# pmeletis/IV2019-boosting-semantic-segmentation-with-weak-labels

Hardware: NVIDIA B200
Metric: train_images_per_s (higher is better)
Workload: dtype bf16

## Files before the change

include/wlseg.h:

```cpp
#ifndef WLSEG_H_
#define WLSEG_H_

#include <stddef.h>
#include <stdint.h>

#ifdef __cplusplus
extern "C" {
#endif

#define WLSEG_VERSION 100

typedef void* wlseg_stream_t;

enum { WLSEG_F32 = 0, WLSEG_BF16 = 1 };
enum { WLSEG_ALGO_AUTO = 0, WLSEG_ALGO_DIRECT = 1, WLSEG_ALGO_TCGEN05 = 2 };

int wlseg_version(void);
const char* wlseg_last_error(void);

typedef struct wlseg_conv_params {
  int32_t N, H, W, C;
  int32_t K, R, S;
  int32_t P, Q;
  int32_t stride, dilation;
// ... 59 lines not shown

int wlseg_bn_finalize_apply(const double* sum, const double* sqsum, int64_t count, int32_t C,
                            const float* gamma, const float* beta, float eps, float decay,
                            float* moving_mean, float* moving_var, float* scale, float* shift,
                            float* saved_mean, float* saved_invstd, const void* z, const void* residual,
                            void* y, uint8_t* relu_mask, int32_t relu, int32_t dtype, wlseg_stream_t stream);

int wlseg_bn_apply(const void* z, const float* scale, const float* shift, const void* residual,
                   void* y, int64_t count, int32_t C, int32_t relu, int32_t dtype,
                   wlseg_stream_t stream);

int wlseg_bn_apply_mask(const void* z, const float* scale, const float* shift, const void* residual,
                        void* y, uint8_t* relu_mask, int64_t count, int32_t C, int32_t dtype,
                        wlseg_stream_t stream);

int wlseg_bn_bwd_reduce(const void* dy, const void* y, const void* z, const float* mean,
                        const float* invstd, const float* scale, const float* shift, int64_t count,
                        int32_t C, int32_t pitch, int32_t relu, int32_t dtype, double* dgamma,
                        double* dbeta, wlseg_stream_t stream);
int wlseg_bn_bwd_apply(const void* dy, const void* y, const void* z, const float* mean,
                       const float* invstd, const float* gamma, const float* scale, const float* shift,
                       const double* dgamma, const double* dbeta, int64_t count, int64_t stat_count,
                       int32_t C, int32_t pitch, int32_t relu, int32_t dtype, void* dz, void* dres,
                       wlseg_stream_t stream);

int wlseg_maxpool_same_fwd(const void* x, void* y, uint8_t* argmax, int32_t N, int32_t H, int32_t W,
                           int32_t C, int32_t ksize, int32_t stride, int32_t dtype,
                           wlseg_stream_t stream);
int wlseg_maxpool_same_bwd(const void* x, const uint8_t* argmax, const void* dy, void* dx, int32_t N,
                           int32_t H, int32_t W, int32_t C, int32_t ksize, int32_t stride,
                           int32_t dtype, wlseg_stream_t stream);

int wlseg_gn_finalize(const double* sum, const double* sqsum, int32_t N, int32_t C, int32_t groups, int64_t hw,
                      const float* gamma, const float* beta, float eps, float* scale, float* shift, float* mean,
                      float* invstd, wlseg_stream_t stream);
int wlseg_gn_bwd_finalize(const double* dgamma_nc, const double* dbeta_nc, int32_t N, int32_t C, int32_t groups,
                          int64_t hw, const float* gamma, const float* mean, const float* invstd, float* cA,
                          float* c1, float* c0, double* dgamma, double* dbeta, wlseg_stream_t stream);
int wlseg_gn_bwd_apply(const void* dy, const void* y, const void* z, const float* cA, const float* c1,
                       const float* c0, const float* scale, const float* shift, int32_t N, int64_t hw, int32_t C,
                       int32_t relu, int32_t dtype, void* dz, void* dres, wlseg_stream_t stream);

int wlseg_avgpool_valid_fwd(const void* x, void* y, int32_t N, int32_t H, int32_t W, int32_t C, int32_t kh,
// ... 106 lines not shown
```

iv2019-boosting-semantic-segmentation-with-weak-labels_b200/csrc/bn.cu:

```cuda
#include <cstdlib>

#include "common.cuh"

namespace wlseg {

static int env_int(const char* name, int dflt) {
  const char* e = getenv(name);
  return e ? atoi(e) : dflt;
}

constexpr int kBnThreads = 256;
constexpr int kBnUnroll = 4;

template <typename T, bool kBackward>
__global__ void __launch_bounds__(kBnThreads)
bn_reduce_kernel(const T* __restrict__ a, const T* __restrict__ yact, const T* __restrict__ z,
                 const float* __restrict__ mean, const float* __restrict__ invstd, const float* __restrict__ scale,
                 const float* __restrict__ shift, int64_t count, int C, int pitch, int relu,
                 double* __restrict__ out0, double* __restrict__ out1, int cspan, int rev) {
  extern __shared__ float part[];
  pdl_launch_dependents();
  pdl_wait();
  if (cspan < C) {
    const int cb = blockIdx.y * cspan;
// ... 290 lines not shown
struct BnFin {
  const double* sum;
  const double* sqsum;
  const float* gamma;
  const float* beta;
  float* moving_mean;
  float* moving_var;
  float* scale_out;
  float* shift_out;
  float* saved_mean;
  float* saved_invstd;
  int64_t count;
  float eps, decay;
};

template <typename T, int kRowsU>
__global__ void __launch_bounds__(256)
bn_apply_rows_kernel(const T* __restrict__ z, const float* __restrict__ scale, const float* __restrict__ shift,
                     const T* __restrict__ res, T* __restrict__ y, int64_t count, int C, int relu, int rev,
                     uint8_t* __restrict__ relu_mask, const BnFin fin) {
  pdl_launch_dependents();
  pdl_wait();
  const int cv = C / 8;
  const int lanes = 256 / cv;
  const int tx = threadIdx.x % cv, ty = threadIdx.x / cv;
  if (ty >= lanes) return;
  const int c0 = tx * 8;
  float sc[8], sh[8];
  if (fin.sum != nullptr) {
    const double n = (double)fin.count;
    const bool publish = blockIdx.x == 0 && ty == 0;
#pragma unroll
    for (int j = 0; j < 8; ++j) {
      const int c = c0 + j;
      const double m = fin.sum[c] / n;
// ... 9 lines not shown
        fin.saved_mean[c] = mf;
        fin.saved_invstd[c] = inv;
        if (fin.moving_mean != nullptr) {
          const float unbiased = fin.count > 1 ? (float)(var * (n / (n - 1.0))) : vf;
          fin.moving_mean[c] -= (1.0f - fin.decay) * (fin.moving_mean[c] - mf);
          fin.moving_var[c] -= (1.0f - fin.decay) * (fin.moving_var[c] - unbiased);
        }
      }
    }
  } else {
    const float4 sa = *reinterpret_cast<const float4*>(scale + c0), sb = *reinterpret_cast<const float4*>(scale + c0 + 4);
    const float4 ha = *reinterpret_cast<const float4*>(shift + c0), hb = *reinterpret_cast<const float4*>(shift + c0 + 4);
    sc[0] = sa.x; sc[1] = sa.y; sc[2] = sa.z; sc[3] = sa.w; sc[4] = sb.x; sc[5] = sb.y; sc[6] = sb.z; sc[7] = sb.w;
    sh[0] = ha.x; sh[1] = ha.y; sh[2] = ha.z; sh[3] = ha.w; sh[4] = hb.x; sh[5] = hb.y; sh[6] = hb.z; sh[7] = hb.w;
  }
  const int64_t step = (int64_t)gridDim.x * lanes;
  for (int64_t row0 = (int64_t)blockIdx.x * lanes + ty; row0 < count; row0 += step * kRowsU) {
    Vec8<T> v[kRowsU], vr[kRowsU];
#pragma unroll
    for (int u = 0; u < kRowsU; ++u) {
      const int64_t row = row0 + u * step;
      if (row < count) {
        const int64_t r = rev ? count - 1 - row : row;
        v[u].load(z + r * C + c0);
        if (res != nullptr) vr[u].load(res + r * C + c0);
      }
    }
#pragma unroll
    for (int u = 0; u < kRowsU; ++u) {
      int64_t row = row0 + u * step;
      if (row >= count) break;
      if (rev) row = count - 1 - row;
      float f[8];
      v[u].unpack(f);
#pragma unroll
      for (int j = 0; j < 8; ++j) f[j] = f[j] * sc[j] + sh[j];
      if (res != nullptr) {
        float r[8];
        vr[u].unpack(r);
#pragma unroll
        for (int j = 0; j < 8; ++j) f[j] += r[j];
      }
      if (relu) {
#pragma unroll
        for (int j = 0; j < 8; ++j) f[j] = fmaxf(f[j], 0.f);
      }
      Vec8<T> o;
      o.pack(f);
      o.store(y + row * C + c0);
      if (relu_mask != nullptr) {
        uint32_t m = 0;
#pragma unroll
        for (int j = 0; j < 8; ++j) m |= (f[j] > 0.f ? 1u : 0u) << j;
        relu_mask[row * cv + tx] = (uint8_t)m;
// ... 71 lines not shown
      Vec8<T> o;
      o.pack(out);
      o.store(dz + e);
    }
  }
}

static bool bn_rows_enabled() { return getenv("WLSEG_BN_FLAT") == nullptr; }
static int bn_apply_u() { return env_int("WLSEG_BN_APPLY_U", 2); }
static int bn_apply_ctas() { return env_int("WLSEG_BN_APPLY_CTAS", 4); }
static int bn_bwd_u() { return env_int("WLSEG_BN_BWD_U", 2); }
static int bn_bwd_ctas() { return env_int("WLSEG_BN_BWD_CTAS", 2); }

template <typename T>
static void launch_apply_rows(const void* z, const float* scale, const float* shift, const void* res, void* y, int64_t count,
                              int C, int relu, cudaStream_t s, uint8_t* mask = nullptr, const BnFin* finp = nullptr) {
  BnFin fin = {};
  if (finp != nullptr) fin = *finp;
  const int lanes = 256 / (C / 8);
  const int U = res != nullptr ? bn_apply_u() : env_int("WLSEG_BN_APPLY_U_PLAIN", 1);
  const int g = bw_grid(ceil_div(count, (int64_t)lanes * U) * 256, 256,
                        res != nullptr ? bn_apply_ctas() : env_int("WLSEG_BN_APPLY_CTAS_PLAIN", 8));
  const int rev = env_int("WLSEG_BN_APPLY_REV", 1);
  cudaError_t e;
  if (U == 1) e = launch_pdl(bn_apply_rows_kernel<T, 1>, dim3(g), dim3(256), 0, s, (const T*)z, scale, shift, (const T*)res, (T*)y, count, C, relu, rev, mask, fin);
  else if (U == 4) e = launch_pdl(bn_apply_rows_kernel<T, 4>, dim3(g), dim3(256), 0, s, (const T*)z, scale, shift, (const T*)res, (T*)y, count, C, relu, rev, mask, fin);
  else e = launch_pdl(bn_apply_rows_kernel<T, 2>, dim3(g), dim3(256), 0, s, (const T*)z, scale, shift, (const T*)res, (T*)y, count, C, relu, rev, mask, fin);
  (void)e;
}

template <typename T>
static void launch_bwd_apply_rows(const void* dy, const void* y, const void* z, const float* mean, const float* invstd,
                                  const float* gamma, const float* scale, const float* shift, const double* dgamma,
                                  const double* dbeta, int64_t count, int64_t stat_count, int C, int pitch, int relu,
                                  void* dz, void* dres, cudaStream_t s) {
  const int lanes = 256 / (C / 8);
  const int U = bn_bwd_u();
  const int g = bw_grid(ceil_div(count, (int64_t)lanes * U) * 256, 256, bn_bwd_ctas());
#define WLSEG_BWD_ROWS(UU)                                                                                          \
  (void)launch_pdl(bn_bwd_apply_rows_kernel<T, UU>, dim3(g), dim3(256), 0, s, (const T*)dy, (const T*)y, (const T*)z,  \
                   mean, invstd, gamma, scale, shift, dgamma, dbeta, count, stat_count, C, pitch, relu, (T*)dz,        \
                   (T*)dres)
// ... 204 lines not shown
  else
    WLSEG_CHECK_ARG(false, "bn_apply: bad dtype %d", dtype);
  WLSEG_LAUNCH_CHECK();
  return 0;
}

extern "C" int wlseg_bn_apply_mask(const void* z, const float* scale, const float* shift, const void* residual, void* y,
                                   uint8_t* relu_mask, int64_t count, int32_t C, int32_t dtype, wlseg_stream_t stream) {
  if (int e = check_bn_shape(count, C, "bn_apply_mask")) return e;
  if (count == 0) return 0;
  WLSEG_CHECK_ARG(z && scale && shift && y && relu_mask, "bn_apply_mask: null pointer");
  WLSEG_CHECK_ARG(C % 32 == 0 && C <= 2048, "bn_apply_mask: C must be a multiple of 32 and <= 2048 (got %d)", C);
  if (dtype == WLSEG_BF16) launch_apply_rows<__nv_bfloat16>(z, scale, shift, residual, y, count, C, 1, (cudaStream_t)stream, relu_mask);
  else if (dtype == WLSEG_F32) launch_apply_rows<float>(z, scale, shift, residual, y, count, C, 1, (cudaStream_t)stream, relu_mask);
  else WLSEG_CHECK_ARG(false, "bn_apply_mask: bad dtype %d", dtype);
  WLSEG_LAUNCH_CHECK();
  return 0;
}

extern "C" int wlseg_bn_bwd_reduce(const void* dy, const void* y, const void* z, const float* mean,
                                   const float* invstd, const float* scale, const float* shift, int64_t count,
                                   int32_t C, int32_t pitch, int32_t relu, int32_t dtype, double* dgamma,
                                   double* dbeta, wlseg_stream_t stream) {
  if (int e = check_bn_shape(count, C, "bn_bwd_reduce")) return e;
  if (count == 0) return 0;
  WLSEG_CHECK_ARG(dy && z && mean && invstd && dgamma && dbeta && (!relu || y || (scale && shift)),
                  "bn_bwd_reduce: null pointer");
  WLSEG_CHECK_ARG(pitch >= C && (C % 8 != 0 ? pitch == C : pitch % 8 == 0), "bn_bwd_reduce: bad pitch %d", pitch);
  WLSEG_CHECK_ARG(C % 8 == 0 || !relu || y, "bn_bwd_reduce: the small-C path needs y for the ReLU mask");
  if (dtype == WLSEG_BF16)
// ... 64 lines not shown
```

iv2019-boosting-semantic-segmentation-with-weak-labels_b200/csrc/pool.cu:

```cuda
#include <cstdlib>

#include "common.cuh"

namespace wlseg {

struct PoolGeom {
  int N, H, W, C, P, Q, k, stride, pad_t, pad_l;
};

template <typename T>
__global__ void __launch_bounds__(256)
maxpool_fwd_kernel(const T* __restrict__ x, T* __restrict__ y, uint8_t* __restrict__ argmax, PoolGeom g) {
  const int cv = g.C / 8;
  const int64_t total = (int64_t)g.N * g.P * g.Q * cv;
  for (int64_t i = (int64_t)blockIdx.x * blockDim.x + threadIdx.x; i < total; i += (int64_t)gridDim.x * blockDim.x) {
    int c8 = (int)(i % cv);
    int64_t t = i / cv;
    int q = (int)(t % g.Q); t /= g.Q;
    int p = (int)(t % g.P);
    int n = (int)(t / g.P);
    float best[8];
    uint32_t arg[8];
#pragma unroll
    for (int j = 0; j < 8; ++j) { best[j] = -INFINITY; arg[j] = 255u; }
// ... 17 lines not shown
    Vec8<T> o;
    o.pack(best);
    const int64_t oi = (((int64_t)n * g.P + p) * g.Q + q) * g.C + c8 * 8;
    o.store(y + oi);
    if (argmax != nullptr) {
      uint2 packed;
      packed.x = arg[0] | (arg[1] << 8) | (arg[2] << 16) | (arg[3] << 24);
      packed.y = arg[4] | (arg[5] << 8) | (arg[6] << 16) | (arg[7] << 24);
      *reinterpret_cast<uint2*>(argmax + oi) = packed;
    }
  }
}

constexpr int kPoolRun = 4;

template <typename T>
__global__ void __launch_bounds__(256)
maxpool3x3s2_fwd_kernel(const T* __restrict__ x, T* __restrict__ y, uint8_t* __restrict__ argmax, PoolGeom g) {
  const int cv = g.C / 8;
  const int runs = (g.Q + kPoolRun - 1) / kPoolRun;
  const int64_t total = (int64_t)g.N * g.P * runs * cv;
  for (int64_t i = (int64_t)blockIdx.x * blockDim.x + threadIdx.x; i < total; i += (int64_t)gridDim.x * blockDim.x) {
    const int c8 = (int)(i % cv);
    int64_t t = i / cv;
    const int run = (int)(t % runs); t /= runs;
    const int p = (int)(t % g.P);
    const int n = (int)(t / g.P);
    const int q0 = run * kPoolRun;
    const int h0 = p * 2 - g.pad_t;
    const T* base = x + (int64_t)n * g.H * g.W * g.C + c8 * 8;
    Vec8<T> col[3][3];
    bool okc[3], okr[3];
#pragma unroll
    for (int r = 0; r < 3; ++r) okr[r] = (h0 + r >= 0) && (h0 + r < g.H);
    auto load_col = [&](int ww, int slot) {
      okc[slot] = ww >= 0 && ww < g.W;
#pragma unroll
      for (int r = 0; r < 3; ++r)
        if (okc[slot] && okr[r]) col[slot][r].load(base + ((int64_t)(h0 + r) * g.W + ww) * g.C);
    };
    const int w0 = q0 * 2 - g.pad_l;
    load_col(w0, 0);
#pragma unroll
    for (int u = 0; u < kPoolRun; ++u) {
      const int q = q0 + u;
      if (q >= g.Q) break;
      const int ww = q * 2 - g.pad_l;
      load_col(ww + 1, 1);
      load_col(ww + 2, 2);
      float best[8];
      uint32_t arg[8];
#pragma unroll
      for (int j = 0; j < 8; ++j) { best[j] = -INFINITY; arg[j] = 255u; }
#pragma unroll
// ... 209 lines not shown

using namespace wlseg;

extern "C" int wlseg_maxpool_same_fwd(const void* x, void* y, uint8_t* argmax, int32_t N, int32_t H, int32_t W,
                                      int32_t C, int32_t ksize, int32_t stride, int32_t dtype,
                                      wlseg_stream_t stream) {
  PoolGeom g;
  if (int e = make_geom(g, N, H, W, C, ksize, stride)) return e;
  if (N == 0) return 0;
  WLSEG_CHECK_ARG(x && y, "maxpool_fwd: null pointer");
  WLSEG_CHECK_ARG(argmax == nullptr || ksize * ksize < 255, "maxpool_fwd: window too large for the uint8 argmax map");
  if (ksize == 3 && stride == 2 && getenv("WLSEG_POOL_GENERIC") == nullptr) {
    const int64_t items3 = (int64_t)N * g.P * ((g.Q + kPoolRun - 1) / kPoolRun) * (C / 8);
    const int grid3 = bw_grid(items3, 256, 2);
    if (dtype == WLSEG_BF16)
      maxpool3x3s2_fwd_kernel<<<grid3, 256, 0, (cudaStream_t)stream>>>((const __nv_bfloat16*)x, (__nv_bfloat16*)y, argmax, g);
    else if (dtype == WLSEG_F32)
      maxpool3x3s2_fwd_kernel<<<grid3, 256, 0, (cudaStream_t)stream>>>((const float*)x, (float*)y, argmax, g);
    else
      WLSEG_CHECK_ARG(false, "maxpool_fwd: bad dtype %d", dtype);
    WLSEG_LAUNCH_CHECK();
    return 0;
  }
  int64_t items = (int64_t)N * g.P * g.Q * (C / 8);
  int grid = bw_grid(items, 256, 8);
  if (dtype == WLSEG_BF16)
    maxpool_fwd_kernel<<<grid, 256, 0, (cudaStream_t)stream>>>((const __nv_bfloat16*)x, (__nv_bfloat16*)y, argmax, g);
  else if (dtype == WLSEG_F32)
    maxpool_fwd_kernel<<<grid, 256, 0, (cudaStream_t)stream>>>((const float*)x, (float*)y, argmax, g);
  else
    WLSEG_CHECK_ARG(false, "maxpool_fwd: bad dtype %d", dtype);
  WLSEG_LAUNCH_CHECK();
  return 0;
}

extern "C" int wlseg_maxpool_same_bwd(const void* x, const uint8_t* argmax, const void* dy, void* dx, int32_t N,
                                      int32_t H, int32_t W, int32_t C, int32_t ksize, int32_t stride,
                                      int32_t dtype, wlseg_stream_t stream) {
  PoolGeom g;
  if (int e = make_geom(g, N, H, W, C, ksize, stride)) return e;
  if (N == 0) return 0;
  WLSEG_CHECK_ARG((x || argmax) && dy && dx, "maxpool_bwd: null pointer");
  int64_t items = (int64_t)N * H * W * (C / 8);
  int grid = bw_grid(items, 256, 8);
  const bool rows_ok = H <= 65535 && N <= 65535 && getenv("WLSEG_POOL_FLAT") == nullptr;
  const dim3 rgrid((unsigned)ceil_div((int64_t)W * (C / 8), 256), (unsigned)H, (unsigned)N);
// ... 43 lines not shown
```

iv2019-boosting-semantic-segmentation-with-weak-labels_b200/wlseg/network.py:

```python

import math
import os

import torch

from wlseg import arch, ops


def _trunc_normal_(t, std, gen):
  torch.nn.init.trunc_normal_(t, mean=0.0, std=std, a=-2 * std, b=2 * std, generator=gen)


class Params:

  def __init__(self, hier, device, output_stride=8, psp=False, fov=None, upsampling='bilinear', norm='batch'):
    self.hier = hier
    self.device = torch.device(device)
    self.psp = bool(psp)
    self.fov = tuple(fov) if fov and fov[0] > 0 and fov[1] > 0 else None
    if upsampling not in ('bilinear', 'no', 'hybrid'):
      raise ValueError('No such upsampling method.')
    self.upsampling = upsampling
    self.specs = arch.conv_specs(hier.head_widths, output_stride, psp=self.psp, fov=self.fov, upsampling=upsampling)
    self.plain = set(arch.UPSAMPLING_SCOPES) if upsampling == 'hybrid' else set()
# ... 558 lines not shown
               cross_replica=None):
    super().__init__(params, dtype, bn_decay, eps, conv_algo)
    self.ws = TrainWorkspace(params)
    self.cross_replica = cross_replica if (cross_replica and cross_replica[0] >= 1) else None
    self.grad_ready = None
    self.keep = False
    self._flipped = None
    self.fused_bn_finalize = os.environ.get('WLSEG_BN_FUSED_FINALIZE', '0') == '1'
    self.bn_bwd_l2_bytes = 1 << 40
    self._order = {s.scope: i for i, s in enumerate(params.specs)}
    self.wgrad_stream = None
    self._side_keep = []
    self.premask = os.environ.get('WLSEG_RELU_MASK', '1') != '0'
    self.bnb_fuse = os.environ.get('WLSEG_BNB_FUSE', '1') != '0'
    self.fin_in_conv = os.environ.get('WLSEG_BN_FIN_IN_CONV', '0') == '1'

  def _mark_done(self, scope, n_elems):
    if self.grad_ready is None:
      return
    lo = self.p.w_off[scope]
    i = self._order[scope]
    specs = self.p.specs
    while i < len(specs) and self.p.w_off[specs[i].scope] < lo + n_elems:
      self._done[i] = True
      i += 1
    t = self._tail
    while t > 0 and self._done[t - 1]:
      t -= 1
    if t != self._tail:
      self._tail = t
      self.grad_ready(self.p.w_off[specs[t].scope])

  def _layer_fwd(self, x, scope, *, w=None, nch=None, relu=None, residual=None, pad=None, stride=None,
                 dilation=None, out_hw=None, y_f32=False, kind='conv', want_mask=False):
    spec = self.p.by_scope[scope]
    if w is None:
      w = self._weights(scope)
    K = w.shape[0] if nch is None else nch
    if pad is None:
      pt, pl, P, Q = self._geom(spec, x.shape[1], x.shape[2])
      pad, out_hw, stride, dilation = (pt, pl), (P, Q), spec.stride, spec.dilation
    N = x.shape[0]
    count = N * out_hw[0] * out_hw[1]
    ws, off = self.ws, self.p.c_off[scope]
    s1, s2 = ws.view(ws.stat, 0, off, K), ws.view(ws.stat, 1, off, K)
    zdt = torch.float32 if y_f32 else self.dtype
    group = self.p.norm == 'group'
    scale, shift = ws.view(ws.bn, 0, off, K), ws.view(ws.bn, 1, off, K)
    mean, invstd = ws.view(ws.bn, 2, off, K), ws.view(ws.bn, 3, off, K)
    fin = None
    if (self.fin_in_conv and not group and self.cross_replica is None and not self.fused_bn_finalize and not y_f32 and
        self.dtype == torch.bfloat16 and self.conv_algo != ops.ALGO_DIRECT and K % 64 == 0 and x.shape[3] % 8 == 0 and
        x.stride(2) % 8 == 0 and not ops.pdl_enabled()):
      fin = (count, self.p.gamma(scope, K), self.p.beta(scope, K), self.eps, self.bn_decay, self.p.moving_mean(scope, K),
             self.p.moving_var(scope, K), scale, shift, mean, invstd, ws.fin_counter)
    z = self._conv(x, w, stride=stride, dilation=dilation, pad=pad, out_hw=out_hw, y_dtype=zdt,
                   bn_sum=None if group else s1, bn_sqsum=None if group else s2, fin=fin)
    a = torch.empty_like(z)
    do_relu = spec.relu if relu is None else relu
    gn = None
    mask = None
    if group:
      gn = self._gn_forward(z, scope, K, do_relu, residual, a)
    elif self.cross_replica is not None:
      R = self.cross_replica[0]
      both = self._all_reduce_pair(s1, s2)
      ops.bn_finalize(both[:K], both[K:], count * R, K, self.p.gamma(scope, K), self.p.beta(scope, K), self.eps,
                      self.bn_decay, self.p.moving_mean(scope, K), self.p.moving_var(scope, K), scale, shift, mean,
                      invstd, moving_var_factor=(count - 1.0) / count)
      ops.bn_apply(z, scale, shift, residual, a, count, K, do_relu)
    elif self.fused_bn_finalize and K % 8 == 0 and K <= 2048 and z.is_contiguous():
      if want_mask and do_relu and K % 32 == 0:
        mask = torch.empty((count, K // 8), dtype=torch.uint8, device=self.dev)
      ops.bn_finalize_apply(s1, s2, count, K, self.p.gamma(scope, K), self.p.beta(scope, K), self.eps, self.bn_decay,
                            self.p.moving_mean(scope, K), self.p.moving_var(scope, K), scale, shift, mean, invstd,
                            z, residual, a, do_relu, mask=mask)
    else:
      if fin is None:
        ops.bn_finalize(s1, s2, count, K, self.p.gamma(scope, K), self.p.beta(scope, K), self.eps, self.bn_decay,
                        self.p.moving_mean(scope, K), self.p.moving_var(scope, K), scale, shift, mean, invstd)
      if want_mask and do_relu and K % 32 == 0 and K <= 2048 and z.is_contiguous():
        mask = torch.empty((count, K // 8), dtype=torch.uint8, device=self.dev)
      ops.bn_apply(z, scale, shift, residual, a, count, K, do_relu, mask=mask)
    rec = _Rec()
    rec.scope, rec.spec, rec.x, rec.w, rec.z, rec.a = scope, spec, x, w, z, a
    rec.relu, rec.has_res, rec.geom, rec.nch, rec.kind = do_relu, residual is not None, (pad, out_hw, stride, dilation), K, kind
    rec.gn = gn
    rec.mask = mask
    rec.res = residual if self.keep else None
    self.tape[scope] = rec
    return a

  def _gn_forward(self, z, scope, K, relu, residual, a):
    N, P, Q, _ = z.shape
    hw = P * Q
    sums = torch.zeros((2, N, K), dtype=torch.float64, device=self.dev)
    for n in range(N):
      ops.bn_stats(z[n], hw, K, z.stride(2), sums[0, n], sums[1, n])
    coef = torch.empty((4, N, K), dtype=torch.float32, device=self.dev)
    ops.gn_finalize(sums[0], sums[1], N, K, self.p.groups(scope, K), hw, self.p.gamma(scope, K), self.p.beta(scope, K),
                    self.eps, coef[0], coef[1], coef[2], coef[3])
    for n in range(N):
      ops.bn_apply(z[n], coef[0, n], coef[1, n], None if residual is None else residual[n], a[n], hw, K, relu)
    return coef

  def _gn_backward(self, rec, da, scope, K, dgamma, dbeta):
# ... 174 lines not shown
        assert dx.is_contiguous()
        ops.add_inplace(dx, dx_add)
    if self.keep:
      rec.dx = dx
    return dx, dres

  def _root_fwd(self, images):
    scope = f'{arch.RES}/conv1'
    N, H, W, _ = images.shape
    if self.dtype == torch.bfloat16:
      Hs, Ws = (H + 1) // 2, (W + 1) // 2
      packed = torch.empty((N, Hs, Ws, 64), dtype=torch.bfloat16, device=self.dev)
      ops.conv1_pack(images, packed)
      self._root_images = images
      y = self._layer_fwd(packed, scope, w=self.p.conv1_packed_weights(torch.bfloat16), pad=(2, 0), stride=1,
                          dilation=1, out_hw=(Hs, Ws), relu=True, kind='root_packed')
    else:
      y = self._layer_fwd(images.to(self.dtype), scope)
    P, Q = (y.shape[1] + 1) // 2, (y.shape[2] + 1) // 2
    pooled = torch.empty((N, P, Q, 64), dtype=self.dtype, device=self.dev)
    amax = torch.empty((N, P, Q, 64), dtype=torch.uint8, device=self.dev)
    ops.maxpool_same_fwd(y, pooled, 3, 2, argmax=amax)
    self.tape['pool1'] = (y, amax)
    return pooled

  def _root_wgrad(self, rec, dz):
    scope = rec.scope
    N, Hs, Ws, _ = rec.x.shape
    pad, out_hw, stride, dilation = rec.geom
    dw2 = torch.empty((64, 4, 1, 64), dtype=torch.float32, device=self.dev)
    prm = ops.conv_params((N, Hs, Ws, 64), (64, 4, 1, 64), stride=stride, dilation=dilation, pad=pad, out_hw=out_hw,
                          x_pitch=rec.x.stride(2), y_pitch=dz.stride(2), dtype=self.code)
    ops.conv2d_wgrad(prm, rec.x, dz, dw2)
    idx = self.p.conv1_pack_index()
    self._wgrad_view(scope, (64, 7, 7, 3)).copy_(dw2.view(64, 256)[:, idx].view(64, 7, 7, 3))

  def _root_bwd(self, dpool):
    y, amax = self.tape['pool1']
    dy = torch.empty_like(y)
    ops.maxpool_same_bwd(None, dpool, dy, 3, 2, argmax=amax)
    self._layer_bwd(f'{arch.RES}/conv1', dy, need_dx=False)

  def _unit_fwd(self, x, u):
    if u.has_shortcut_conv:
      sc = self._layer_fwd(x, f'{u.scope}/shortcut')
    elif u.stride > 1:
      N, H, W, C = x.shape
      sc = torch.empty((N, (H + u.stride - 1) // u.stride, (W + u.stride - 1) // u.stride, C), dtype=self.dtype,
                       device=self.dev)
      ops.maxpool_same_fwd(x, sc, 1, u.stride)
    else:
      sc = x
    r = self._layer_fwd(x, f'{u.scope}/conv1')
    r = self._layer_fwd(r, f'{u.scope}/conv2')
    self.tape[u.scope] = x
    return self._layer_fwd(r, f'{u.scope}/conv3', relu=True, residual=sc, want_mask=self._use_premask())

  def _use_premask(self):
    return (self.premask and not self.keep and self.dtype == torch.bfloat16 and self.conv_algo != ops.ALGO_DIRECT and
            self.p.norm == 'batch')

  def _unit_bwd(self, dout, u, dout_masked=False, in_mask=None):
    x = self.tape[u.scope]
    c1, c2 = f'{u.scope}/conv1', f'{u.scope}/conv2'
    f2 = self._bnb_args(c2) is not None
    f1 = self._bnb_args(c1) is not None
    dr, dsc = self._layer_bwd(f'{u.scope}/conv3', dout, da_masked=dout_masked, bnb_below=c2 if f2 else None)
    dr, _ = self._layer_bwd(c2, dr, da_reduced=f2, bnb_below=c1 if f1 else None)
    if u.has_shortcut_conv:
      dx, _ = self._layer_bwd(c1, dr, da_reduced=f1)
      dx, _ = self._layer_bwd(f'{u.scope}/shortcut', dsc, dx_add=dx, dx_mask=in_mask)
# ... 151 lines not shown
```

iv2019-boosting-semantic-segmentation-with-weak-labels_b200/wlseg/ops.py:

```python

import ctypes
import os

import torch

_HERE = os.path.dirname(os.path.abspath(__file__))
LIB_PATH = os.path.join(_HERE, 'lib', 'libwlseg.so')

F32, BF16 = 0, 1
ALGO_AUTO, ALGO_DIRECT, ALGO_TCGEN05 = 0, 1, 2

_c_int = ctypes.c_int32
_c_i64 = ctypes.c_int64
_c_f = ctypes.c_float
_vp = ctypes.c_void_p


class WlsegError(RuntimeError):
  pass


class ConvParams(ctypes.Structure):
  _fields_ = [(n, _c_int) for n in (
      'N', 'H', 'W', 'C', 'K', 'R', 'S', 'P', 'Q', 'stride', 'dilation', 'pad_top', 'pad_left',
# ... 20 lines not shown

_SIGNATURES = {
    'wlseg_version': (ctypes.c_int, []),
    'wlseg_last_error': (ctypes.c_char_p, []),
    'wlseg_conv2d_tcgen05_supported': (ctypes.c_int, [ctypes.POINTER(ConvParams)]),
    'wlseg_conv2d_fprop': (ctypes.c_int, [ctypes.POINTER(ConvParams), _vp, _vp, _vp, _vp, _vp, _vp, _vp, _vp, _vp]),
    'wlseg_conv2d_dgrad': (ctypes.c_int, [ctypes.POINTER(ConvParams), _vp, _vp, _vp, _vp]),
    'wlseg_conv2d_wgrad': (ctypes.c_int, [ctypes.POINTER(ConvParams), _vp, _vp, _vp, _vp]),
    'wlseg_bn_stats': (ctypes.c_int, [_vp, _c_i64, _c_int, _c_int, _c_int, _vp, _vp, _vp]),
    'wlseg_bn_finalize': (ctypes.c_int, [_vp, _vp, _c_i64, _c_int, _vp, _vp, _c_f, _c_f, _c_f, _vp, _vp, _vp, _vp, _vp,
                                         _vp, _vp]),
    'wlseg_bn_finalize_apply': (ctypes.c_int, [_vp, _vp, _c_i64, _c_int, _vp, _vp, _c_f, _c_f, _vp, _vp, _vp, _vp, _vp,
                                               _vp, _vp, _vp, _vp, _vp, _c_int, _c_int, _vp]),
    'wlseg_bn_apply': (ctypes.c_int, [_vp, _vp, _vp, _vp, _vp, _c_i64, _c_int, _c_int, _c_int, _vp]),
    'wlseg_bn_apply_mask': (ctypes.c_int, [_vp, _vp, _vp, _vp, _vp, _vp, _c_i64, _c_int, _c_int, _vp]),
    'wlseg_conv2d_fprop_masked': (ctypes.c_int, [ctypes.POINTER(ConvParams), _vp, _vp, _vp, _vp, _vp, _vp]),
    'wlseg_conv2d_fprop_bnbwd': (ctypes.c_int, [ctypes.POINTER(ConvParams)] + [_vp] * 11),
    'wlseg_conv2d_fprop_bn': (ctypes.c_int, [ctypes.POINTER(ConvParams), _vp, _vp, _vp, _vp, _vp,
                                             ctypes.POINTER(BnFinalizeArgs), _vp]),
    'wlseg_bn_bwd_reduce': (ctypes.c_int, [_vp, _vp, _vp, _vp, _vp, _vp, _vp, _c_i64, _c_int, _c_int, _c_int, _c_int,
                                           _vp, _vp, _vp]),
    'wlseg_bn_bwd_apply': (ctypes.c_int, [_vp, _vp, _vp, _vp, _vp, _vp, _vp, _vp, _vp, _vp, _c_i64, _c_i64, _c_int, _c_int,
                                          _c_int, _c_int, _vp, _vp, _vp]),
    'wlseg_maxpool_same_fwd': (ctypes.c_int, [_vp, _vp, _vp, _c_int, _c_int, _c_int, _c_int, _c_int, _c_int, _c_int,
                                              _vp]),
    'wlseg_maxpool_same_bwd': (ctypes.c_int, [_vp, _vp, _vp, _vp, _c_int, _c_int, _c_int, _c_int, _c_int, _c_int,
                                              _c_int, _vp]),
    'wlseg_gn_finalize': (ctypes.c_int, [_vp, _vp, _c_int, _c_int, _c_int, _c_i64, _vp, _vp, _c_f, _vp, _vp, _vp, _vp, _vp]),
    'wlseg_gn_bwd_finalize': (ctypes.c_int, [_vp, _vp, _c_int, _c_int, _c_int, _c_i64] + [_vp] * 9),
    'wlseg_gn_bwd_apply': (ctypes.c_int, [_vp] * 8 + [_c_int, _c_i64, _c_int, _c_int, _c_int, _vp, _vp, _vp]),
    'wlseg_avgpool_valid_fwd': (ctypes.c_int, [_vp, _vp] + [_c_int] * 9 + [_vp]),
    'wlseg_avgpool_valid_bwd': (ctypes.c_int, [_vp, _vp] + [_c_int] * 8 + [_vp]),
    'wlseg_resize_bilinear_fwd': (ctypes.c_int, [_vp, _vp] + [_c_int] * 8 + [_vp]),
    'wlseg_resize_bilinear_bwd': (ctypes.c_int, [_vp, _vp] + [_c_int] * 8 + [_vp]),
    'wlseg_rasterize_bbox_labels': (ctypes.c_int, [_vp, _vp, _c_int, _c_int, _c_int, _c_int, _vp, _vp]),
    'wlseg_tile_image_labels': (ctypes.c_int, [_vp, _c_int, _c_int, _c_int, _vp, _vp]),
    'wlseg_head_fwd': (ctypes.c_int, [ctypes.POINTER(Hierarchy), _vp, _c_int, _c_int, _c_int, _c_int, _c_int, _c_int,
                                      _vp, _vp, _vp, _vp, _vp, _vp, _vp, _vp, _vp]),
    'wlseg_resize_probabilities': (ctypes.c_int, [_vp, _vp] + [_c_int] * 6 + [_vp]),
    'wlseg_resize_decisions': (ctypes.c_int, [_vp, _vp] + [_c_int] * 5 + [_vp]),
# ... 230 lines not shown


def bn_apply(z, scale, shift, residual, y, count, C, relu, mask=None):
  if mask is not None:
    assert relu and mask.dtype == torch.uint8 and mask.numel() == count * (C // 8)
    _count()
    _check(lib().wlseg_bn_apply_mask(_ptr(z), _ptr(scale), _ptr(shift), _ptr(residual), _ptr(y), _ptr(mask), count, C,
                                     dtype_code(z.dtype), _stream()), 'wlseg_bn_apply_mask')
    return
  _check(lib().wlseg_bn_apply(_ptr(z), _ptr(scale), _ptr(shift), _ptr(residual), _ptr(y), count, C, int(relu),
                              dtype_code(z.dtype), _stream()), 'wlseg_bn_apply')
  _count()
  return y


def bn_bwd_reduce(dy, y, z, mean, invstd, count, C, relu, dgamma, dbeta, scale=None, shift=None, pitch=None):
  _check(lib().wlseg_bn_bwd_reduce(_ptr(dy), _ptr(y), _ptr(z), _ptr(mean), _ptr(invstd), _ptr(scale), _ptr(shift),
                                   count, C, C if pitch is None else pitch, int(relu), dtype_code(z.dtype),
                                   _ptr(dgamma), _ptr(dbeta), _stream()), 'wlseg_bn_bwd_reduce')
  _count()


def bn_bwd_apply(dy, y, z, mean, invstd, gamma, dgamma, dbeta, count, C, relu, dz, dres=None, scale=None, shift=None,
                 pitch=None, stat_count=None):
  _check(lib().wlseg_bn_bwd_apply(_ptr(dy), _ptr(y), _ptr(z), _ptr(mean), _ptr(invstd), _ptr(gamma), _ptr(scale),
                                  _ptr(shift), _ptr(dgamma), _ptr(dbeta), count, count if stat_count is None else stat_count,
                                  C, C if pitch is None else pitch,
                                  int(relu), dtype_code(z.dtype), _ptr(dz), _ptr(dres), _stream()),
         'wlseg_bn_bwd_apply')
  _count()
# ... 13 lines not shown
  _count()


def gn_bwd_apply(dy, y, z, cA, c1, c0, scale, shift, N, hw, C, relu, dz, dres=None):
  assert dy.is_contiguous() and z.is_contiguous() and dz.is_contiguous()
  _check(lib().wlseg_gn_bwd_apply(_ptr(dy), _ptr(y), _ptr(z), _ptr(cA), _ptr(c1), _ptr(c0), _ptr(scale), _ptr(shift), N, hw,
                                  C, int(relu), dtype_code(z.dtype), _ptr(dz), _ptr(dres), _stream()), 'wlseg_gn_bwd_apply')
  _count()
  return dz


def maxpool_same_fwd(x, y, ksize, stride, argmax=None):
  N, H, W, C = x.shape
  _check(lib().wlseg_maxpool_same_fwd(_ptr(x), _ptr(y), _ptr(argmax), N, H, W, C, ksize, stride,
                                      dtype_code(x.dtype), _stream()), 'wlseg_maxpool_same_fwd')
  _count()
  return y


def maxpool_same_bwd(x, dy, dx, ksize, stride, argmax=None):
  N, H, W, C = dx.shape
  _check(lib().wlseg_maxpool_same_bwd(_ptr(x), _ptr(argmax), _ptr(dy), _ptr(dx), N, H, W, C, ksize, stride,
                                      dtype_code(dx.dtype), _stream()), 'wlseg_maxpool_same_bwd')
  _count()
  return dx


def avgpool_valid_fwd(x, y, kh, kw):
  N, H, W, C = x.shape
  assert x.is_contiguous() and y.is_contiguous() and tuple(y.shape) == (N, (H - kh) // kh + 1, (W - kw) // kw + 1, C)
# ... 268 lines not shown
```

Before: 378.0.

## Defer BN apply into consumers: fuse root BN+ReLU into maxpool and shortcut BN into residual

Adds a deferred-BN path where a conv returns its raw output plus scale/shift instead of writing a normalized activation. The root conv's BN+ReLU is applied inside the 3x3/s2 maxpool kernel, and the shortcut conv's BN is applied inside the conv3 residual-add/mask kernel. This removes a full read-write pass over two large activation tensors per use, in exchange for redundant BN arithmetic on overlapping pool windows and extra per-channel loads. Backward is left unchanged, so it relies on the tape holding z and scale/shift in a form the existing backward still handles correctly.

```diff
diff --git a/include/wlseg.h b/include/wlseg.h
--- a/include/wlseg.h
+++ b/include/wlseg.h
@@ -97,6 +97,10 @@
                         void* y, uint8_t* relu_mask, int64_t count, int32_t C, int32_t dtype,
                         wlseg_stream_t stream);
 
+int wlseg_bn_apply_mask_bnres(const void* z, const float* scale, const float* shift, const void* residual,
+                              const float* residual_scale, const float* residual_shift, void* y, uint8_t* relu_mask,
+                              int64_t count, int32_t C, int32_t dtype, wlseg_stream_t stream);
+
 int wlseg_bn_bwd_reduce(const void* dy, const void* y, const void* z, const float* mean,
                         const float* invstd, const float* scale, const float* shift, int64_t count,
                         int32_t C, int32_t pitch, int32_t relu, int32_t dtype, double* dgamma,
@@ -110,6 +114,9 @@
 int wlseg_maxpool_same_fwd(const void* x, void* y, uint8_t* argmax, int32_t N, int32_t H, int32_t W,
                            int32_t C, int32_t ksize, int32_t stride, int32_t dtype,
                            wlseg_stream_t stream);
+int wlseg_maxpool_same_fwd_bnrelu(const void* z, const float* scale, const float* shift, void* y, uint8_t* argmax,
+                                  int32_t N, int32_t H, int32_t W, int32_t C, int32_t ksize, int32_t stride,
+                                  int32_t dtype, wlseg_stream_t stream);
 int wlseg_maxpool_same_bwd(const void* x, const uint8_t* argmax, const void* dy, void* dx, int32_t N,
                            int32_t H, int32_t W, int32_t C, int32_t ksize, int32_t stride,
                            int32_t dtype, wlseg_stream_t stream);
diff --git a/iv2019-boosting-semantic-segmentation-with-weak-labels_b200/csrc/bn.cu b/iv2019-boosting-semantic-segmentation-with-weak-labels_b200/csrc/bn.cu
--- a/iv2019-boosting-semantic-segmentation-with-weak-labels_b200/csrc/bn.cu
+++ b/iv2019-boosting-semantic-segmentation-with-weak-labels_b200/csrc/bn.cu
@@ -328,11 +328,12 @@
   float eps, decay;
 };
 
-template <typename T, int kRowsU>
+template <typename T, int kRowsU, bool kResBn = false>
 __global__ void __launch_bounds__(256)
 bn_apply_rows_kernel(const T* __restrict__ z, const float* __restrict__ scale, const float* __restrict__ shift,
                      const T* __restrict__ res, T* __restrict__ y, int64_t count, int C, int relu, int rev,
-                     uint8_t* __restrict__ relu_mask, const BnFin fin) {
+                     uint8_t* __restrict__ relu_mask, const BnFin fin, const float* __restrict__ rscale,
+                     const float* __restrict__ rshift) {
   pdl_launch_dependents();
   pdl_wait();
   const int cv = C / 8;
@@ -372,6 +373,11 @@
     sc[0] = sa.x; sc[1] = sa.y; sc[2] = sa.z; sc[3] = sa.w; sc[4] = sb.x; sc[5] = sb.y; sc[6] = sb.z; sc[7] = sb.w;
     sh[0] = ha.x; sh[1] = ha.y; sh[2] = ha.z; sh[3] = ha.w; sh[4] = hb.x; sh[5] = hb.y; sh[6] = hb.z; sh[7] = hb.w;
   }
+  float rsc[8], rsh[8];
+  if (kResBn) {
+#pragma unroll
+    for (int j = 0; j < 8; ++j) { rsc[j] = rscale[c0 + j]; rsh[j] = rshift[c0 + j]; }
+  }
   const int64_t step = (int64_t)gridDim.x * lanes;
   for (int64_t row0 = (int64_t)blockIdx.x * lanes + ty; row0 < count; row0 += step * kRowsU) {
     Vec8<T> v[kRowsU], vr[kRowsU];
@@ -396,6 +402,13 @@
       if (res != nullptr) {
         float r[8];
         vr[u].unpack(r);
+        if (kResBn) {
+#pragma unroll
+          for (int j = 0; j < 8; ++j) r[j] = fmaf(r[j], rsc[j], rsh[j]);
+          Vec8<T> t;
+          t.pack(r);
+          t.unpack(r);
+        }
 #pragma unroll
         for (int j = 0; j < 8; ++j) f[j] += r[j];
       }
@@ -497,7 +510,8 @@
 
 template <typename T>
 static void launch_apply_rows(const void* z, const float* scale, const float* shift, const void* res, void* y, int64_t count,
-                              int C, int relu, cudaStream_t s, uint8_t* mask = nullptr, const BnFin* finp = nullptr) {
+                              int C, int relu, cudaStream_t s, uint8_t* mask = nullptr, const BnFin* finp = nullptr,
+                              const float* rscale = nullptr, const float* rshift = nullptr) {
   BnFin fin = {};
   if (finp != nullptr) fin = *finp;
   const int lanes = 256 / (C / 8);
@@ -506,9 +520,10 @@
                         res != nullptr ? bn_apply_ctas() : env_int("WLSEG_BN_APPLY_CTAS_PLAIN", 8));
   const int rev = env_int("WLSEG_BN_APPLY_REV", 1);
   cudaError_t e;
-  if (U == 1) e = launch_pdl(bn_apply_rows_kernel<T, 1>, dim3(g), dim3(256), 0, s, (const T*)z, scale, shift, (const T*)res, (T*)y, count, C, relu, rev, mask, fin);
-  else if (U == 4) e = launch_pdl(bn_apply_rows_kernel<T, 4>, dim3(g), dim3(256), 0, s, (const T*)z, scale, shift, (const T*)res, (T*)y, count, C, relu, rev, mask, fin);
-  else e = launch_pdl(bn_apply_rows_kernel<T, 2>, dim3(g), dim3(256), 0, s, (const T*)z, scale, shift, (const T*)res, (T*)y, count, C, relu, rev, mask, fin);
+  if (rscale != nullptr) e = launch_pdl(bn_apply_rows_kernel<T, 2, true>, dim3(g), dim3(256), 0, s, (const T*)z, scale, shift, (const T*)res, (T*)y, count, C, relu, rev, mask, fin, rscale, rshift);
+  else if (U == 1) e = launch_pdl(bn_apply_rows_kernel<T, 1>, dim3(g), dim3(256), 0, s, (const T*)z, scale, shift, (const T*)res, (T*)y, count, C, relu, rev, mask, fin, rscale, rshift);
+  else if (U == 4) e = launch_pdl(bn_apply_rows_kernel<T, 4>, dim3(g), dim3(256), 0, s, (const T*)z, scale, shift, (const T*)res, (T*)y, count, C, relu, rev, mask, fin, rscale, rshift);
+  else e = launch_pdl(bn_apply_rows_kernel<T, 2>, dim3(g), dim3(256), 0, s, (const T*)z, scale, shift, (const T*)res, (T*)y, count, C, relu, rev, mask, fin, rscale, rshift);
   (void)e;
 }
 
@@ -743,6 +758,25 @@
   if (dtype == WLSEG_BF16) launch_apply_rows<__nv_bfloat16>(z, scale, shift, residual, y, count, C, 1, (cudaStream_t)stream, relu_mask);
   else if (dtype == WLSEG_F32) launch_apply_rows<float>(z, scale, shift, residual, y, count, C, 1, (cudaStream_t)stream, relu_mask);
   else WLSEG_CHECK_ARG(false, "bn_apply_mask: bad dtype %d", dtype);
+  WLSEG_LAUNCH_CHECK();
+  return 0;
+}
+
+extern "C" int wlseg_bn_apply_mask_bnres(const void* z, const float* scale, const float* shift, const void* residual,
+                                         const float* residual_scale, const float* residual_shift, void* y,
+                                         uint8_t* relu_mask, int64_t count, int32_t C, int32_t dtype, wlseg_stream_t stream) {
+  if (int e = check_bn_shape(count, C, "bn_apply_mask_bnres")) return e;
+  if (count == 0) return 0;
+  WLSEG_CHECK_ARG(z && scale && shift && residual && residual_scale && residual_shift && y && relu_mask,
+                  "bn_apply_mask_bnres: null pointer");
+  WLSEG_CHECK_ARG(C % 32 == 0 && C <= 2048, "bn_apply_mask_bnres: C must be a multiple of 32 and <= 2048 (got %d)", C);
+  if (dtype == WLSEG_BF16)
+    launch_apply_rows<__nv_bfloat16>(z, scale, shift, residual, y, count, C, 1, (cudaStream_t)stream, relu_mask, nullptr,
+                                     residual_scale, residual_shift);
+  else if (dtype == WLSEG_F32)
+    launch_apply_rows<float>(z, scale, shift, residual, y, count, C, 1, (cudaStream_t)stream, relu_mask, nullptr,
+                             residual_scale, residual_shift);
+  else WLSEG_CHECK_ARG(false, "bn_apply_mask_bnres: bad dtype %d", dtype);
   WLSEG_LAUNCH_CHECK();
   return 0;
 }
diff --git a/iv2019-boosting-semantic-segmentation-with-weak-labels_b200/csrc/pool.cu b/iv2019-boosting-semantic-segmentation-with-weak-labels_b200/csrc/pool.cu
--- a/iv2019-boosting-semantic-segmentation-with-weak-labels_b200/csrc/pool.cu
+++ b/iv2019-boosting-semantic-segmentation-with-weak-labels_b200/csrc/pool.cu
@@ -55,9 +55,10 @@
 
 constexpr int kPoolRun = 4;
 
-template <typename T>
-__global__ void __launch_bounds__(256)
-maxpool3x3s2_fwd_kernel(const T* __restrict__ x, T* __restrict__ y, uint8_t* __restrict__ argmax, PoolGeom g) {
+template <typename T, bool kBn>
+__global__ void __launch_bounds__(256)
+maxpool3x3s2_fwd_kernel(const T* __restrict__ x, T* __restrict__ y, uint8_t* __restrict__ argmax, PoolGeom g,
+                        const float* __restrict__ scale, const float* __restrict__ shift) {
   const int cv = g.C / 8;
   const int runs = (g.Q + kPoolRun - 1) / kPoolRun;
   const int64_t total = (int64_t)g.N * g.P * runs * cv;
@@ -70,6 +71,11 @@
     const int q0 = run * kPoolRun;
     const int h0 = p * 2 - g.pad_t;
     const T* base = x + (int64_t)n * g.H * g.W * g.C + c8 * 8;
+    float sc[8], sh[8];
+    if (kBn) {
+#pragma unroll
+      for (int j = 0; j < 8; ++j) { sc[j] = scale[c8 * 8 + j]; sh[j] = shift[c8 * 8 + j]; }
+    }
     Vec8<T> col[3][3];
     bool okc[3], okr[3];
 #pragma unroll
@@ -78,7 +84,16 @@
       okc[slot] = ww >= 0 && ww < g.W;
 #pragma unroll
       for (int r = 0; r < 3; ++r)
-        if (okc[slot] && okr[r]) col[slot][r].load(base + ((int64_t)(h0 + r) * g.W + ww) * g.C);
+        if (okc[slot] && okr[r]) {
+          col[slot][r].load(base + ((int64_t)(h0 + r) * g.W + ww) * g.C);
+          if (kBn) {
+            float f[8];
+            col[slot][r].unpack(f);
+#pragma unroll
+            for (int j = 0; j < 8; ++j) f[j] = fmaxf(fmaf(f[j], sc[j], sh[j]), 0.f);
+            col[slot][r].pack(f);
+          }
+        }
     };
     const int w0 = q0 * 2 - g.pad_l;
     load_col(w0, 0);
@@ -318,9 +333,11 @@
     const int64_t items3 = (int64_t)N * g.P * ((g.Q + kPoolRun - 1) / kPoolRun) * (C / 8);
     const int grid3 = bw_grid(items3, 256, 2);
     if (dtype == WLSEG_BF16)
-      maxpool3x3s2_fwd_kernel<<<grid3, 256, 0, (cudaStream_t)stream>>>((const __nv_bfloat16*)x, (__nv_bfloat16*)y, argmax, g);
+      maxpool3x3s2_fwd_kernel<__nv_bfloat16, false><<<grid3, 256, 0, (cudaStream_t)stream>>>(
+          (const __nv_bfloat16*)x, (__nv_bfloat16*)y, argmax, g, nullptr, nullptr);
     else if (dtype == WLSEG_F32)
-      maxpool3x3s2_fwd_kernel<<<grid3, 256, 0, (cudaStream_t)stream>>>((const float*)x, (float*)y, argmax, g);
+      maxpool3x3s2_fwd_kernel<float, false><<<grid3, 256, 0, (cudaStream_t)stream>>>((const float*)x, (float*)y, argmax, g,
+                                                                                     nullptr, nullptr);
     else
       WLSEG_CHECK_ARG(false, "maxpool_fwd: bad dtype %d", dtype);
     WLSEG_LAUNCH_CHECK();
@@ -334,6 +351,29 @@
     maxpool_fwd_kernel<<<grid, 256, 0, (cudaStream_t)stream>>>((const float*)x, (float*)y, argmax, g);
   else
     WLSEG_CHECK_ARG(false, "maxpool_fwd: bad dtype %d", dtype);
+  WLSEG_LAUNCH_CHECK();
+  return 0;
+}
+
+extern "C" int wlseg_maxpool_same_fwd_bnrelu(const void* z, const float* scale, const float* shift, void* y,
+                                             uint8_t* argmax, int32_t N, int32_t H, int32_t W, int32_t C, int32_t ksize,
+                                             int32_t stride, int32_t dtype, wlseg_stream_t stream) {
+  PoolGeom g;
+  if (int e = make_geom(g, N, H, W, C, ksize, stride)) return e;
+  WLSEG_CHECK_ARG(ksize == 3 && stride == 2, "maxpool_fwd_bnrelu: only the 3x3 / stride-2 window (got %d / %d)", ksize,
+                  stride);
+  if (N == 0) return 0;
+  WLSEG_CHECK_ARG(z && scale && shift && y, "maxpool_fwd_bnrelu: null pointer");
+  const int64_t items3 = (int64_t)N * g.P * ((g.Q + kPoolRun - 1) / kPoolRun) * (C / 8);
+  const int grid3 = bw_grid(items3, 256, 2);
+  if (dtype == WLSEG_BF16)
+    maxpool3x3s2_fwd_kernel<__nv_bfloat16, true><<<grid3, 256, 0, (cudaStream_t)stream>>>(
+        (const __nv_bfloat16*)z, (__nv_bfloat16*)y, argmax, g, scale, shift);
+  else if (dtype == WLSEG_F32)
+    maxpool3x3s2_fwd_kernel<float, true><<<grid3, 256, 0, (cudaStream_t)stream>>>((const float*)z, (float*)y, argmax, g,
+                                                                                  scale, shift);
+  else
+    WLSEG_CHECK_ARG(false, "maxpool_fwd_bnrelu: bad dtype %d", dtype);
   WLSEG_LAUNCH_CHECK();
   return 0;
 }
diff --git a/iv2019-boosting-semantic-segmentation-with-weak-labels_b200/wlseg/network.py b/iv2019-boosting-semantic-segmentation-with-weak-labels_b200/wlseg/network.py
--- a/iv2019-boosting-semantic-segmentation-with-weak-labels_b200/wlseg/network.py
+++ b/iv2019-boosting-semantic-segmentation-with-weak-labels_b200/wlseg/network.py
@@ -596,6 +596,8 @@
     self.premask = os.environ.get('WLSEG_RELU_MASK', '1') != '0'
     self.bnb_fuse = os.environ.get('WLSEG_BNB_FUSE', '1') != '0'
     self.fin_in_conv = os.environ.get('WLSEG_BN_FIN_IN_CONV', '0') == '1'
+    self.bn_at_consumer = (os.environ.get('WLSEG_BN_AT_CONSUMER', '1') != '0' and
+                           torch.device(params.device).type == 'cuda')
 
   def _mark_done(self, scope, n_elems):
     if self.grad_ready is None:
@@ -614,7 +616,8 @@
       self.grad_ready(self.p.w_off[specs[t].scope])
 
   def _layer_fwd(self, x, scope, *, w=None, nch=None, relu=None, residual=None, pad=None, stride=None,
-                 dilation=None, out_hw=None, y_f32=False, kind='conv', want_mask=False):
+                 dilation=None, out_hw=None, y_f32=False, kind='conv', want_mask=False, defer_bn=False,
+                 residual_bn=None):
     spec = self.p.by_scope[scope]
     if w is None:
       w = self._weights(scope)
@@ -638,11 +641,20 @@
              self.p.moving_var(scope, K), scale, shift, mean, invstd, ws.fin_counter)
     z = self._conv(x, w, stride=stride, dilation=dilation, pad=pad, out_hw=out_hw, y_dtype=zdt,
                    bn_sum=None if group else s1, bn_sqsum=None if group else s2, fin=fin)
-    a = torch.empty_like(z)
+    a = None if defer_bn else torch.empty_like(z)
     do_relu = spec.relu if relu is None else relu
     gn = None
     mask = None
-    if group:
+    if defer_bn or residual_bn is not None:
+      assert not group and self.cross_replica is None and not self.fused_bn_finalize
+      if fin is None:
+        ops.bn_finalize(s1, s2, count, K, self.p.gamma(scope, K), self.p.beta(scope, K), self.eps, self.bn_decay,
+                        self.p.moving_mean(scope, K), self.p.moving_var(scope, K), scale, shift, mean, invstd)
+      if residual_bn is not None:
+        assert want_mask and do_relu and K % 32 == 0 and K <= 2048 and z.is_contiguous()
+        mask = torch.empty((count, K // 8), dtype=torch.uint8, device=self.dev)
+        ops.bn_apply_mask_bnres(z, scale, shift, residual, residual_bn[0], residual_bn[1], a, mask, count, K)
+    elif group:
       gn = self._gn_forward(z, scope, K, do_relu, residual, a)
     elif self.cross_replica is not None:
       R = self.cross_replica[0]
@@ -671,7 +683,11 @@
     rec.mask = mask
     rec.res = residual if self.keep else None
     self.tape[scope] = rec
-    return a
+    return (z, scale, shift) if defer_bn else a
+
+  def _defer_bn(self):
+    return (self.bn_at_consumer and not self.keep and self.dtype == torch.bfloat16 and self.conv_algo != ops.ALGO_DIRECT
+            and self.p.norm == 'batch' and self.cross_replica is None and not self.fused_bn_finalize)
 
   def _gn_forward(self, z, scope, K, relu, residual, a):
     N, P, Q, _ = z.shape
@@ -876,13 +892,19 @@
       ops.conv1_pack(images, packed)
       self._root_images = images
       y = self._layer_fwd(packed, scope, w=self.p.conv1_packed_weights(torch.bfloat16), pad=(2, 0), stride=1,
-                          dilation=1, out_hw=(Hs, Ws), relu=True, kind='root_packed')
+                          dilation=1, out_hw=(Hs, Ws), relu=True, kind='root_packed', defer_bn=self._defer_bn())
     else:
       y = self._layer_fwd(images.to(self.dtype), scope)
+    bn = None
+    if isinstance(y, tuple):
+      y, *bn = y
     P, Q = (y.shape[1] + 1) // 2, (y.shape[2] + 1) // 2
     pooled = torch.empty((N, P, Q, 64), dtype=self.dtype, device=self.dev)
     amax = torch.empty((N, P, Q, 64), dtype=torch.uint8, device=self.dev)
-    ops.maxpool_same_fwd(y, pooled, 3, 2, argmax=amax)
+    if bn is None:
+      ops.maxpool_same_fwd(y, pooled, 3, 2, argmax=amax)
+    else:
+      ops.maxpool_same_fwd_bnrelu(y, bn[0], bn[1], pooled, 3, 2, argmax=amax)
     self.tape['pool1'] = (y, amax)
     return pooled
 
@@ -904,7 +926,11 @@
     self._layer_bwd(f'{arch.RES}/conv1', dy, need_dx=False)
 
   def _unit_fwd(self, x, u):
-    if u.has_shortcut_conv:
+    premask = self._use_premask()
+    sc_bn = None
+    if u.has_shortcut_conv and premask and self._defer_bn():
+      sc, *sc_bn = self._layer_fwd(x, f'{u.scope}/shortcut', defer_bn=True)
+    elif u.has_shortcut_conv:
       sc = self._layer_fwd(x, f'{u.scope}/shortcut')
     elif u.stride > 1:
       N, H, W, C = x.shape
@@ -916,7 +942,7 @@
     r = self._layer_fwd(x, f'{u.scope}/conv1')
     r = self._layer_fwd(r, f'{u.scope}/conv2')
     self.tape[u.scope] = x
-    return self._layer_fwd(r, f'{u.scope}/conv3', relu=True, residual=sc, want_mask=self._use_premask())
+    return self._layer_fwd(r, f'{u.scope}/conv3', relu=True, residual=sc, want_mask=premask, residual_bn=sc_bn)
 
   def _use_premask(self):
     return (self.premask and not self.keep and self.dtype == torch.bfloat16 and self.conv_algo != ops.ALGO_DIRECT and
diff --git a/iv2019-boosting-semantic-segmentation-with-weak-labels_b200/wlseg/ops.py b/iv2019-boosting-semantic-segmentation-with-weak-labels_b200/wlseg/ops.py
--- a/iv2019-boosting-semantic-segmentation-with-weak-labels_b200/wlseg/ops.py
+++ b/iv2019-boosting-semantic-segmentation-with-weak-labels_b200/wlseg/ops.py
@@ -58,6 +58,7 @@
                                                _vp, _vp, _vp, _vp, _vp, _c_int, _c_int, _vp]),
     'wlseg_bn_apply': (ctypes.c_int, [_vp, _vp, _vp, _vp, _vp, _c_i64, _c_int, _c_int, _c_int, _vp]),
     'wlseg_bn_apply_mask': (ctypes.c_int, [_vp, _vp, _vp, _vp, _vp, _vp, _c_i64, _c_int, _c_int, _vp]),
+    'wlseg_bn_apply_mask_bnres': (ctypes.c_int, [_vp] * 8 + [_c_i64, _c_int, _c_int, _vp]),
     'wlseg_conv2d_fprop_masked': (ctypes.c_int, [ctypes.POINTER(ConvParams), _vp, _vp, _vp, _vp, _vp, _vp]),
     'wlseg_conv2d_fprop_bnbwd': (ctypes.c_int, [ctypes.POINTER(ConvParams)] + [_vp] * 11),
     'wlseg_conv2d_fprop_bn': (ctypes.c_int, [ctypes.POINTER(ConvParams), _vp, _vp, _vp, _vp, _vp,
@@ -68,6 +69,7 @@
                                           _c_int, _c_int, _vp, _vp, _vp]),
     'wlseg_maxpool_same_fwd': (ctypes.c_int, [_vp, _vp, _vp, _c_int, _c_int, _c_int, _c_int, _c_int, _c_int, _c_int,
                                               _vp]),
+    'wlseg_maxpool_same_fwd_bnrelu': (ctypes.c_int, [_vp] * 5 + [_c_int] * 7 + [_vp]),
     'wlseg_maxpool_same_bwd': (ctypes.c_int, [_vp, _vp, _vp, _vp, _c_int, _c_int, _c_int, _c_int, _c_int, _c_int,
                                               _c_int, _vp]),
     'wlseg_gn_finalize': (ctypes.c_int, [_vp, _vp, _c_int, _c_int, _c_int, _c_i64, _vp, _vp, _c_f, _vp, _vp, _vp, _vp, _vp]),
@@ -328,6 +330,15 @@
   return y
 
 
+def bn_apply_mask_bnres(z, scale, shift, residual, residual_scale, residual_shift, y, mask, count, C):
+  assert mask.dtype == torch.uint8 and mask.numel() == count * (C // 8)
+  _check(lib().wlseg_bn_apply_mask_bnres(_ptr(z), _ptr(scale), _ptr(shift), _ptr(residual), _ptr(residual_scale),
+                                         _ptr(residual_shift), _ptr(y), _ptr(mask), count, C, dtype_code(z.dtype),
+                                         _stream()), 'wlseg_bn_apply_mask_bnres')
+  _count()
+  return y
+
+
 def bn_bwd_reduce(dy, y, z, mean, invstd, count, C, relu, dgamma, dbeta, scale=None, shift=None, pitch=None):
   _check(lib().wlseg_bn_bwd_reduce(_ptr(dy), _ptr(y), _ptr(z), _ptr(mean), _ptr(invstd), _ptr(scale), _ptr(shift),
                                    count, C, C if pitch is None else pitch, int(relu), dtype_code(z.dtype),
@@ -371,6 +382,14 @@
   N, H, W, C = x.shape
   _check(lib().wlseg_maxpool_same_fwd(_ptr(x), _ptr(y), _ptr(argmax), N, H, W, C, ksize, stride,
                                       dtype_code(x.dtype), _stream()), 'wlseg_maxpool_same_fwd')
+  _count()
+  return y
+
+
+def maxpool_same_fwd_bnrelu(z, scale, shift, y, ksize, stride, argmax=None):
+  N, H, W, C = z.shape
+  _check(lib().wlseg_maxpool_same_fwd_bnrelu(_ptr(z), _ptr(scale), _ptr(shift), _ptr(y), _ptr(argmax), N, H, W, C, ksize,
+                                             stride, dtype_code(z.dtype), _stream()), 'wlseg_maxpool_same_fwd_bnrelu')
   _count()
   return y
 
```

Result: no change. 380.0 (median of 6 runs) (+0.5%).
